# ZSHCRWY25/3DRVO-MARL-CollisionAvoidance

Hardware: AMD Instinct MI355X
Metric: drone-steps/sec (env.step throughput) (higher is better)
Workload: dtype f64; 1 GPU; BASELINE config 3 env.step: 64 drones x 4096 envs per GPU, nm=10, 0 buildings, map [50.0, 50.0, 10.0], fused step+auto-reset, f32 actions in HBM; envs_per_gpu=4096, drones=64, diag_build=False, cold_all=False, ablate=0, device_error_word=0

## Files before the change

3drvo-marl-collisionavoidance_amd/csrc/rvo3d_aux_kernels.hpp:

```cpp
#pragma once

#include "rvo3d_step.hpp"
#include "rvo3d_rvo_rules.hpp"

namespace rvo3d {

__device__ __forceinline__ void reset_drone(const Params& P, int g) {
  double s[3];
  load_wp(P, g, 0, s);
  P.px()[g] = s[0]; P.py()[g] = s[1]; P.pz()[g] = s[2];
  P.vx()[g] = 0.0; P.vy()[g] = 0.0; P.vz()[g] = 0.0;
  P.wp_idx()[g] = 1; P.arrive()[g] = 0; P.dest()[g] = 0;
  P.real_len()[g] = 0.0; P.max_dev()[g] = 0.0; P.yaw()[g] = 0.0; P.pitch()[g] = 0.0;
  double c1[3];
  load_wp(P, g, 1, c1);
  store3(P.cur(0), P.cur(1), P.cur(2), g, c1);
  store3(P.prev(0), P.prev(1), P.prev(2), g, s);
  const bool plain = P.dev0()[g] == 0.0;
  P.dvk_a()[g] = plain ? P.dv0_a()[g] : kDvInvalid;
  P.dvk_b()[g] = P.dv0_b()[g];
}
__global__ void reset_kernel(const Params P, const uint8_t* env_mask, const uint8_t* drone_mask) {
  const int g = blockIdx.x * blockDim.x + threadIdx.x;
  if (g >= P.E * P.N) return;
  if (env_mask && !env_mask[g / P.N]) return;
  if (drone_mask && !drone_mask[g]) return;
  reset_drone(P, g);
}

__global__ void reset_fresh_kernel(const Params P, const uint8_t* env_mask) {
  const int g = blockIdx.x * blockDim.x + threadIdx.x;
  if (g >= P.E * P.N) return;
  if (!env_mask[g / P.N]) return;
  reset_drone(P, g);
  P.extra_len()[g] = 0.0;
}

__global__ void wpcache_kernel(const Params P) {
  const int g = blockIdx.x * blockDim.x + threadIdx.x;
  if (g >= P.E * P.N) return;
  const int np = P.n_points()[g];
  int i = P.wp_idx()[g];
  i = i < 1 ? 1 : (i > np - 1 ? np - 1 : i);
  double v[3];
  load_wp(P, g, i, v);
  store3(P.cur(0), P.cur(1), P.cur(2), g, v);
  load_wp(P, g, i - 1, v);
  store3(P.prev(0), P.prev(1), P.prev(2), g, v);
}

__device__ __forceinline__ void dv0_drone(const Params& P, int g) {
  double p[3], cur[3], dv[3];
  load_wp(P, g, 0, p);
  load_wp(P, g, 1, cur);
  des_vel(P, p, cur, dv);
  uint32_t a, b;
  dv_encode(dv, a, b);
  P.dv0_a()[g] = a; P.dv0_b()[g] = b;
  P.dev0()[g] = deviation(p, cur, p);
}
__global__ void dv0_kernel(const Params P) {
  const int g = blockIdx.x * blockDim.x + threadIdx.x;
  if (g >= P.E * P.N) return;
  dv0_drone(P, g);
}

__device__ __forceinline__ int live_drones(const Params& P, int e) { return P.cold().counts[e]; }

template <bool CNT>
__device__ __forceinline__ void des_vel_body(const Params P, double* out) {
  const int g = blockIdx.x * blockDim.x + threadIdx.x;
  if (g >= P.E * P.N) return;
  if (CNT) {
    const int e = g / P.N;
    if (g - e * P.N >= live_drones(P, e)) {
      out[3 * (size_t)g] = 0.0; out[3 * (size_t)g + 1] = 0.0; out[3 * (size_t)g + 2] = 0.0;
      return;
    }
  }
  double p[3] = {P.px()[g], P.py()[g], P.pz()[g]}, cur[3], dv[3];
  load3(P.cur(0), P.cur(1), P.cur(2), g, cur);
  des_vel(P, p, cur, dv);
  out[3 * (size_t)g] = dv[0]; out[3 * (size_t)g + 1] = dv[1]; out[3 * (size_t)g + 2] = dv[2];
}
__global__ void des_vel_kernel(const Params P, double* out) { des_vel_body<false>(P, out); }
__global__ void des_vel_counted_kernel(const Params P, double* out) { des_vel_body<true>(P, out); }

struct RvoVelArgs { double vmax[3]; double acceler; };

__device__ __forceinline__ int arange_len(double lo, double hi) {
  const double n = __builtin_ceil((hi - lo) / 0.5);
  return n > 0 ? (int)n : 0;
}
__device__ __forceinline__ double arange_at(double lo, int k) {
  const double next = lo + 0.5;
  return k == 0 ? lo : (k == 1 ? next : lo + k * (next - lo));
}


__device__ __forceinline__ unsigned long long rvo_grid(const RvoVelArgs& A, const double* v0, double* lo, int* cnt) {
#pragma unroll
  for (int k = 0; k < 3; ++k) {
    lo[k] = clampd(v0[k] - A.acceler, -A.vmax[k], A.vmax[k]);
    const double hi = clampd(v0[k] + A.acceler, -A.vmax[k], A.vmax[k]);
    cnt[k] = arange_len(lo[k], hi);
    if (cnt[k] > 4) cnt[k] = 4;
  }
  unsigned long long live = 0ull;
  int c = 0;
  for (int ix = 0; ix < cnt[0]; ++ix)
    for (int iy = 0; iy < cnt[1]; ++iy)
      for (int iz = 0; iz < cnt[2]; ++iz, ++c)
// ... 134 lines not shown
```

3drvo-marl-collisionavoidance_amd/csrc/rvo3d_host_setup.hpp:

```cpp
#pragma once

#include "../../include/rvo3d.h"
#include "rvo3d_params.hpp"
#include "rvo3d_lds.hpp"

#include <cmath>
#include <cstring>
#include <string>
#include <vector>

namespace rvo3d {

inline size_t align_up(size_t x, size_t a) { return (x + a - 1) / a * a; }
inline volatile double kTwo = 2.0;
inline double py_sq(double x) { return std::pow(x, kTwo); }

inline double sq_threshold(double tau) {
  volatile double x = tau * tau;
  while (std::sqrt(std::nextafter((double)x, INFINITY)) <= tau) x = std::nextafter((double)x, INFINITY);
  while (std::sqrt((double)x) > tau) x = std::nextafter((double)x, -INFINITY);
  return x;
}

struct Pick { int nfix; bool pad; };
// ... 113 lines not shown
  two_phase = epb == P.epb && out.threads == G.threads;
  return RVO3D_OK;
}

inline int zero_fill_tables(const Params& P, int threads, Cold& C, std::string& err) {
  const int N = P.N, epb = P.epb;
  C.zf_div = (uint32_t)((P.W & 1) == 0 ? (P.W - 12) / 2 : (P.W - 12));
  C.zf_magic = 0;
  if (C.zf_div > 0) {
    const uint32_t m = (uint32_t)(((1ull << 32) + C.zf_div - 1) / C.zf_div);
    bool ok = true;
    const uint64_t qmax = (uint64_t)threads * C.zf_div;
    for (uint64_t q = 0; q < qmax && ok; ++q) ok = ((q * m) >> 32) == q / C.zf_div;
    if (!ok) {
      err = "neighbors_num too large for the zero-fill index trick";
      return RVO3D_ERR_INVALID;
    }
    C.zf_magic = m;
  }
  C.zf_q = (P.W & 1) == 0 ? (uint32_t)(P.W / 2) : 0u;
  C.zf_iters = 0;
  static_assert(kMaxThreads / 4 <= sizeof(C.zmask) / sizeof(C.zmask[0]),
                "Cold::zmask has one word per thread quad of the largest workgroup");
  std::memset(C.zmask, 0, sizeof C.zmask);
  {
    const uint32_t rb = 4u * (uint32_t)P.W;
    const uint32_t rows_full = (uint32_t)epb * (uint32_t)N, nwv = (uint32_t)threads / 64u;
    const uint32_t nblk = rows_full * rb >> 6;
    const uint32_t iters = (nblk + 16u * nwv - 1u) / (16u * nwv);
    if (C.zf_q != 0 && P.W >= 48 && (rows_full & 7u) == 0 && iters <= 32u) {
      for (uint32_t tq = 0; tq < (uint32_t)threads / 4u; ++tq) {
        uint32_t m = 0;
        for (uint32_t i = 0; i < iters; ++i) {
          const uint32_t blk = tq + 16u * nwv * i;
          if (blk >= nblk) break;
          const uint32_t o = (blk * 64u) % rb;
          if (o >= 48u && o + 64u <= rb) m |= 1u << i;
        }
        C.zmask[tq] = m;
      }
      C.zf_iters = (int)iters;
    }
  }
  return RVO3D_OK;
}

inline int plan_env(const rvo3d_config* cfg, int lds_pad, Params& P, Cold& C, Geometry& G, std::string& err) {
  std::memset(&P, 0, sizeof P);
  std::memset(&C, 0, sizeof C);
  P.E = cfg->num_envs; P.N = cfg->num_drones; P.P = cfg->max_points;
  C.nb = cfg->num_buildings; P.nm = cfg->neighbors_num; P.env_train = cfg->env_train ? 1 : 0;
  P.W = 12 + 9 * P.nm;
  C.act_scale = cfg->action_decimals >= 0 ? std::pow(10.0, cfg->action_decimals) : 0.0;
  for (int k = 0; k < 3; ++k) C.map[k] = cfg->map_size[k];
  P.T10 = sq_threshold(10.0);
  C.T5 = sq_threshold(5.0);
  building_grid_dims(cfg, C);
  C.T04 = sq_threshold(0.4);
  filter_bands(P, C);
  if (int rc = launch_geometry(lds_pad, P, G, err)) return rc;
  return zero_fill_tables(P, G.threads, C, err);
}

struct StagedWorld { std::vector<double> wp, rl, rad, pri, p95; };
inline int stage_world(Params& P, const double* waypoints, const int32_t* n_points, const double* radius,
                       const double* priority, StagedWorld& w, std::string& err) {
  const size_t EN = (size_t)P.E * P.N;
  std::vector<double> wp((size_t)P.P * 3 * EN), rl(EN), rad(EN), pri(EN), p95(P.P);
  for (size_t g = 0; g < EN; ++g) {
    const int np = n_points[g];
    if (np < 2 || np > P.P) {
      err = "n_points entries must be in [2, max_points]";
      return RVO3D_ERR_INVALID;
    }
    const double* src = waypoints + g * P.P * 3;
    double total = 0.0;
    for (int k = 0; k < P.P; ++k) {
      const int kk = k < np ? k : np - 1;
      for (int c = 0; c < 3; ++c) wp[((size_t)k * 3 + c) * EN + g] = src[kk * 3 + c];
      if (k + 1 < np) {
        const double dx = src[(k + 1) * 3] - src[k * 3], dy = src[(k + 1) * 3 + 1] - src[k * 3 + 1],
                     dz = src[(k + 1) * 3 + 2] - src[k * 3 + 2];
        total += std::sqrt(py_sq(dx) + py_sq(dy) + py_sq(dz));
      }
    }
    rl[g] = total;
    rad[g] = radius ? radius[g] : 0.2;
    pri[g] = priority ? priority[g] : 5.0;
  }
  {
    bool uni = true;
    for (size_t g = 1; g < EN && uni; ++g)
      uni = std::memcmp(&rad[g], &rad[0], 8) == 0 && std::memcmp(&pri[g], &pri[0], 8) == 0;
    P.uniform_rp = uni ? 1 : 0;
    P.r0 = rad[0];
    P.prio0 = pri[0];
  }
  for (int k = 0; k < P.P; ++k) p95[k] = std::pow(0.95, (double)k);
  w.wp.swap(wp); w.rl.swap(rl); w.rad.swap(rad); w.pri.swap(pri); w.p95.swap(p95);
  return RVO3D_OK;
}

inline double largest_radius(const std::vector<double>& rad) {
  double rmax = 0.0;
  for (size_t g = 0; g < rad.size(); ++g) {
    if (rad[g] != rad[g]) rmax = INFINITY;
// ... 161 lines not shown
```

3drvo-marl-collisionavoidance_amd/csrc/rvo3d_math.hpp:

```cpp
#pragma once

#include "rvo3d_params.hpp"

namespace rvo3d {

__device__ __forceinline__ double sq(double x) { return x * x; }
__device__ __forceinline__ double dot3b(double ax, double ay, double az, double bx,
                                        double by, double bz) {
  return __builtin_fma(az, bz, __builtin_fma(ay, by, ax * bx));
}
__device__ __forceinline__ double norm3b(double x, double y, double z) {
  return __builtin_sqrt(dot3b(x, y, z, x, y, z));
}
__device__ __forceinline__ double norm2sq(double x, double y) { return __builtin_fma(y, y, x * x); }
__device__ __forceinline__ bool finite_d(double q) { return __builtin_fabs(q) < __builtin_inf(); }

__device__ __forceinline__ float round2_f32(double x) {
  const double k = __builtin_rint(x * 100.0);
  return __builtin_fabs(k) < 16777216.0 ? (float)(k * 0.01) : (float)(k / 100.0);
}
__device__ __forceinline__ double k_over_1000(double k) {
  const double q = k * 0.001;
  const double r = __builtin_fma(-q, 1000.0, k);
  const double c = q + r * 0.001;
  return finite_d(k) ? c : k;
}

constexpr uint32_t kDvInvalid = 0xffffffffu;
__device__ __forceinline__ void dv_encode(const double dv[3], uint32_t& a, uint32_t& b) {
  const double k0 = __builtin_rint(dv[0] * 1000.0), k1 = __builtin_rint(dv[1] * 1000.0),
               k2 = __builtin_rint(dv[2] * 1000.0);
  const bool ok = __builtin_fabs(k0) <= 1023.0 && __builtin_fabs(k1) <= 1023.0 &&
                  __builtin_fabs(k2) <= 1023.0 && k_over_1000(k0) == dv[0] &&
                  k_over_1000(k1) == dv[1] && k_over_1000(k2) == dv[2];
  const uint32_t nz = (uint32_t)(k0 == 0.0 && __builtin_signbit(dv[0])) |
                      ((uint32_t)(k1 == 0.0 && __builtin_signbit(dv[1])) << 1) |
                      ((uint32_t)(k2 == 0.0 && __builtin_signbit(dv[2])) << 2);
  a = ok ? ((uint32_t)((int)k0 + 1024) | ((uint32_t)((int)k1 + 1024) << 16)) : kDvInvalid;
  b = (uint32_t)((int)(ok ? k2 : 0.0) + 1024) | (nz << 16);
}
__device__ __forceinline__ bool dv_decode(uint32_t a, uint32_t b, double dv[3]) {
  if (a == kDvInvalid) return false;
  const int k0 = (int)(a & 0xffffu) - 1024, k1 = (int)(a >> 16) - 1024, k2 = (int)(b & 0xffffu) - 1024;
  dv[0] = (b & (1u << 16)) ? -0.0 : k_over_1000((double)k0);
  dv[1] = (b & (1u << 17)) ? -0.0 : k_over_1000((double)k1);
  dv[2] = (b & (1u << 18)) ? -0.0 : k_over_1000((double)k2);
  return true;
}

__device__ __forceinline__ double py_round2_c(double x) {
  double p = x * 100.0;
  double e = __builtin_fma(x, 100.0, -p);
  double c = __builtin_floor(p);
  double d = (p - (c + 0.5)) + e;
  if (d > 0.0) c += 1.0;
  else if (d == 0.0 && (((long long)c) & 1)) c += 1.0;
  return c;
}
__device__ __forceinline__ double clampd(double x, double lo, double hi) {
  return x < lo ? lo : (x > hi ? hi : x);
}
__device__ __forceinline__ double np_mod(double a, double b) {
  double m;
  if (b > 0.0 && a > -b && a < 2.0 * b) m = a >= b ? a - b : a;
  else m = fmod(a, b);
  if (m != 0.0) {
    if ((b < 0.0) != (m < 0.0)) m += b;
  } else {
    m = __builtin_copysign(0.0, b);
  }
  return m;
}

__device__ __forceinline__ void des_vel(double T04, const double p[3], const double cur[3], double out[3]) {
  const double dx = cur[0] - p[0], dy = cur[1] - p[1], dz = cur[2] - p[2];
  const double d2 = dot3b(dx, dy, dz, dx, dy, dz);
  if (d2 > T04) {
    const double inv = 1000.0 / __builtin_sqrt(d2);
    const double ux = dx * inv, uy = dy * inv, uz = dz * inv;
    double kx = __builtin_rint(ux), ky = __builtin_rint(uy), kz = __builtin_rint(uz);
    const double m = __builtin_fmin(__builtin_fmin(0.5 - __builtin_fabs(ux - kx),
                                                   0.5 - __builtin_fabs(uy - ky)),
                                    0.5 - __builtin_fabs(uz - kz));
    if (!(m > 1e-7)) {
      const double az = atan2(dy, dx);
      const double el = atan2(dz, __builtin_sqrt(norm2sq(dx, dy)));
      double sa, ca, se, ce;
      sincos(az, &sa, &ca);
      sincos(el, &se, &ce);
      kx = __builtin_rint((1.0 * (ca * ce)) * 1000.0);
      ky = __builtin_rint((1.0 * (sa * ce)) * 1000.0);
      kz = __builtin_rint((1.0 * se) * 1000.0);
    }
    out[0] = k_over_1000(kx); out[1] = k_over_1000(ky); out[2] = k_over_1000(kz);
  } else {
    out[0] = out[1] = out[2] = 0.0;
  }
}
__device__ __forceinline__ void des_vel(const Params& P, const double p[3], const double cur[3],
                                        double out[3]) {
  des_vel(P.cold().T04, p, cur, out);
}

__device__ __forceinline__ double deviation(const double a[3], const double b[3],
                                            const double p[3]) {
  double dx = b[0] - a[0], dy = b[1] - a[1], dz = b[2] - a[2];
  double mag = __builtin_sqrt(sq(dx) + sq(dy) + sq(dz));
  if (mag == 0.0) return 0.0;
  double hx = dx / mag, hy = dy / mag, hz = dz / mag;
  double qx0 = p[0] - a[0], qy0 = p[1] - a[1], qz0 = p[2] - a[2];
  double t = qx0 * hx + qy0 * hy + qz0 * hz;
  double qx = a[0] + t * hx, qy = a[1] + t * hy, qz = a[2] + t * hz;
  return __builtin_sqrt(sq(p[0] - qx) + sq(p[1] - qy) + sq(p[2] - qz));
}

__device__ __forceinline__ bool arrived(double T04, const double p[3], const double d[3]) {
  const double x = p[0] - d[0], y = p[1] - d[1], z = p[2] - d[2];
  return dot3b(x, y, z, x, y, z) <= T04;
}

__device__ __forceinline__ double vo_exp_time(double rx, double ry, double rz, double rvx,
                                              double rvy, double rvz, double ra, double rb) {
  double r = ra + rb;
  double ux = -rvx, uy = -rvy, uz = -rvz;
  double a = sq(ux) + sq(uy) + sq(uz);
  double b = 2 * rx * ux + 2 * ry * uy + 2 * rz * uz;
  double c = sq(rx) + sq(ry) + sq(rz) - sq(r);
  if (c <= 0) return 0.0;
  double temp = sq(b) - 4 * a * c;
  if (temp <= 0) return __builtin_inf();
  double s = __builtin_sqrt(temp);
  double t1 = (-b + s) / (2 * a);
  double t2 = (-b - s) / (2 * a);
  if (t1 < 0 && t2 < 0) return -1.0;
  double t3 = t1 >= 0 ? t1 : __builtin_inf();
  double t4 = t2 >= 0 ? t2 : __builtin_inf();
  return t4 < t3 ? t4 : t3;
}

struct Drone {
  double x, y, z, vx, vy, vz, r, prio;
};

struct PairOut {
  bool collision, flag;
  double t, iet, md;
  int alpha_c;
};

}
```

3drvo-marl-collisionavoidance_amd/csrc/rvo3d_params.hpp:

```cpp
#pragma once

#include <hip/hip_runtime.h>
#include <stdint.h>

namespace rvo3d {

constexpr double kExpRadius = 0.2;
constexpr double kCtimeThreshold = 2.0;
constexpr double kDeg2Rad = 0.017453292519943295;
constexpr double kPi = 3.141592653589793;
constexpr int kMaxThreads = 512;
constexpr double kCosD = 0.999999995;
constexpr double kSinD = 1.0000000000e-4;

struct Cold {
  double map[3];
  double T5, T04;
  double cen[3];
  double act_scale;
  float cmax;
  float kdot;
  uint32_t zf_div;
  uint32_t zf_magic;
  uint32_t zf_q;
  int zf_iters;
  uint32_t zmask[128];
  int nb;
  const double* bld;
  const double* pow95;
  const uint16_t* bgrid;
  int bgx, bgy;
  double bg_inv;
  uint32_t bld_stride, bgrid_stride;
  const int32_t* counts;
  int cnt_two_phase;
};
constexpr int kBgridK = 15;
typedef const __attribute__((address_space(4))) Cold ColdC;

struct Params {
  int E, N, P, nm, env_train, epb, W;
  int action_f64;
  int dv_cached;
  int g_cached;
  int action_mode;
  float acceler;
#ifdef RVO3D_DIAG
  int ablate;
#endif
  int zf16;
  int uniform_rp;
  double r0, prio0;
  double T10;
  float t10n;
  float bandn;
  float band;
  int nw;
  float x1_gap;
  float x1_k2;
  float x1_cs2;
  double* f64;
  int32_t* i32;
  uint8_t* u8;
  uint32_t S;
  enum { F_PX, F_PY, F_PZ, F_VX, F_VY, F_VZ, F_YAW, F_PITCH, F_REAL_LEN, F_MAX_DEV, F_EXTRA_LEN,
         F_CUR, F_PREV = F_CUR + 3,
         F_ROUTE_LEN = F_PREV + 3, F_RADIUS, F_PRIO, F_DEV0, F_WP };
  __host__ __device__ double* f(int k) const { return f64 + (size_t)k * S; }
  __host__ __device__ double* px() const { return f(F_PX); }
  __host__ __device__ double* py() const { return f(F_PY); }
  __host__ __device__ double* pz() const { return f(F_PZ); }
  __host__ __device__ double* vx() const { return f(F_VX); }
  __host__ __device__ double* vy() const { return f(F_VY); }
  __host__ __device__ double* vz() const { return f(F_VZ); }
  __host__ __device__ double* yaw() const { return f(F_YAW); }
  __host__ __device__ double* pitch() const { return f(F_PITCH); }
  __host__ __device__ double* real_len() const { return f(F_REAL_LEN); }
  __host__ __device__ double* max_dev() const { return f(F_MAX_DEV); }
  __host__ __device__ double* extra_len() const { return f(F_EXTRA_LEN); }
  __host__ __device__ int32_t* wp_idx() const { return i32; }
  __host__ __device__ uint8_t* arrive() const { return u8; }
  __host__ __device__ uint8_t* dest() const { return u8 + S; }
  __host__ __device__ double* route_len() const { return f(F_ROUTE_LEN); }
  __host__ __device__ double* radius() const { return f(F_RADIUS); }
  __host__ __device__ double* prio() const { return f(F_PRIO); }
  __host__ __device__ double* dev0() const { return f(F_DEV0); }
  __host__ __device__ double* wp(int k, int c) const { return f(F_WP + 3 * k + c); }
  __host__ __device__ double* cur(int c) const { return f(F_CUR + c); }
  __host__ __device__ double* prev(int c) const { return f(F_PREV + c); }
  __host__ __device__ int32_t* n_points() const { return i32 + S; }
  __host__ __device__ uint32_t* dvk_a() const { return reinterpret_cast<uint32_t*>(i32) + (size_t)2 * S; }
  __host__ __device__ uint32_t* dvk_b() const { return reinterpret_cast<uint32_t*>(i32) + (size_t)3 * S; }
  __host__ __device__ uint32_t* dv0_a() const { return reinterpret_cast<uint32_t*>(i32) + (size_t)4 * S; }
  __host__ __device__ uint32_t* dv0_b() const { return reinterpret_cast<uint32_t*>(i32) + (size_t)5 * S; }
  __host__ __device__ uint32_t* gcache(int w) const { return reinterpret_cast<uint32_t*>(i32) + (size_t)(6 + w) * S; }
  __host__ __device__ double* row_iet(int s) const { return f(F_WP + 3 * P + s); }
  __host__ __device__ uint32_t* row_pk(int s) const {
    return reinterpret_cast<uint32_t*>(i32) + (size_t)(6 + nw + s) * S;
  }
  __host__ __device__ static size_t f64_arrays(int P_, int nm_) { return F_WP + 3 * (size_t)P_ + (nm_ > 0 ? nm_ : 1); }
  __host__ __device__ static size_t i32_arrays(int nm_, int nw_) { return 6 + (size_t)nw_ + (size_t)(nm_ > 0 ? nm_ : 1); }
  uint32_t* err;
  const Cold* cold_;
  __device__ __forceinline__ ColdC& cold() const { return *(ColdC*)cold_; }
#ifdef RVO3D_DIAG
  unsigned long long* dbg;
#endif
  const void* actions;
  float* obs;
  int32_t* vo_count;
  float* reward;
  double* reward64;
  uint8_t *done, *info, *finish, *reset_mask;
  const int32_t* prev_cnt;
};

#ifdef RVO3D_DIAG
#define RVO3D_STAMP(i)                                                                  \
  do {                                                                                  \
    if (P.dbg && threadIdx.x == 0) P.dbg[(size_t)blockIdx.x * 32 + (i)] = __builtin_amdgcn_s_memtime(); \
  } while (0)
#define RVO3D_ABLATED(bits) ((P.ablate & (bits)) != 0)
#else
#define RVO3D_STAMP(i) do { } while (0)
#define RVO3D_ABLATED(bits) false
#endif

}
```

3drvo-marl-collisionavoidance_amd/csrc/rvo3d_step.hpp:

```cpp
#pragma once

#include "rvo3d_pairs.hpp"

namespace rvo3d {

__device__ __forceinline__ bool building_test(const double* const bld, int b, const Drone& S,
                                              double T5) {
  const double bx = bld[4 * b], by = bld[4 * b + 1], bh = bld[4 * b + 2], br = bld[4 * b + 3];
  const double ex = S.x - bx, ey = S.y - by;
  if ((bh > S.z - 2) & (norm2sq(ex, ey) <= T5) & (S.z <= bh))
    return __builtin_sqrt(sq(ex) + sq(ey)) <= S.r + br;
  return false;
}
__device__ __forceinline__ bool building_hit(const Params& P, const Drone& S, int e) {
  const int nb = P.cold().nb;
  if (nb == 0) return false;
  bool hit = false;
  const double* const bld = P.cold().bld + (size_t)e * P.cold().bld_stride;
  const double T5 = P.cold().T5;
  const int gx = P.cold().bgx;
  if (gx > 0) {
    const int gy = P.cold().bgy;
    const double inv = P.cold().bg_inv;
    int ix = (int)__builtin_floor(S.x * inv), iy = (int)__builtin_floor(S.y * inv);
// ... 167 lines not shown
#pragma unroll
    for (int u = 0; u < 4; ++u)
      if ((m >> u) & 1u) {
        *reinterpret_cast<v4f*>(p + u * step) = (v4f){0.f, 0.f, 0.f, 0.f};
      }
  }
}

template <int NW>
__device__ __forceinline__ void late_row_windows(const Params& P, const Lds& L, int tid, int row0,
                                                 int nrows) {
  const uint32_t rb = 4u * (uint32_t)P.W, q = rb >> 3;
  const int ln = tid & 63, wv = tid >> 6;
  const int nwv = waves_of<NW>(L);
  const float2* pro2 = reinterpret_cast<const float2*>(L.w[0]);
  char* const base = reinterpret_cast<char*>(P.obs) + (size_t)row0 * rb;
  const int ch = ln & 7;
  const int r0 = wv * 8 + (ln >> 3);
  const uint32_t rs0 = rb * (uint32_t)r0;
  const uint32_t s8 = (rs0 & 63u) >> 3;
  const uint32_t ua = 2u * (uint32_t)ch, ub = ua + 1u;
  const bool pa = ua < s8, pb = ub < s8;
  const uint32_t uia = pa ? q - s8 + ua : ua - s8, uib = pb ? q - s8 + ub : ub - s8;
  const bool proa = uia < 6u, prob = uib < 6u;
  const int pia = (int)(proa ? uia : 5u), pib = (int)(prob ? uib : 5u);
  const int da_row = pa ? 1 : 0, db_row = pb ? 1 : 0;
  char* pc = base + (rs0 & ~63u) + 16u * (uint32_t)ch;
  const size_t step = (size_t)8 * (size_t)nwv * rb;
  for (int r = r0; r < nrows; r += 8 * nwv, pc += step) {
    const int ra = r - da_row, rbw = r - db_row;
    const int za = L.kept[ra], zb = L.kept[rbw];
    const float2 da = pro2[ra * 6 + pia], db = pro2[rbw * 6 + pib];
    const bool va = proa | (uia >= (uint32_t)za), vb = prob | (uib >= (uint32_t)zb);
    const float2 a = proa ? da : make_float2(0.f, 0.f), b = prob ? db : make_float2(0.f, 0.f);
    if (va & vb) *reinterpret_cast<float4*>(pc) = make_float4(a.x, a.y, b.x, b.y);
    if (va != vb) *reinterpret_cast<float2*>(pc + (vb ? 8 : 0)) = vb ? b : a;
  }
}

__device__ __forceinline__ void write_vo_rows(const Params& P, const Lds& L, int tid, int lbase,
                                              int g, const Drone& S, int kept) {
  float* o = P.obs + (size_t)g * P.W;
  bool bad = false;
  for (int s = 0; s < kept; ++s) {
    const uint32_t pk = P.row_pk(s)[g];
    const int j = (int)(pk & 0xffffu);
    const Drone O = lds_drone(L, lbase + j);
    const double pr = (S.prio == O.prio) ? 0.5 : S.prio / (S.prio + O.prio);
    double row[9];
    row[0] = pr * (2 * S.x + (S.vx + O.vx));
    row[1] = pr * (2 * S.y + (S.vy + O.vy));
    row[2] = pr * (2 * S.z + (S.vz + O.vz));
    row[3] = O.x - S.x; row[4] = O.y - S.y; row[5] = O.z - S.z;
    row[6] = (double)(pk >> 16) / 100.0;
    row[7] = pair_md(S, O);
    row[8] = P.row_iet(s)[g];
#pragma unroll
    for (int k = 0; k < 9; ++k) {
      bad |= !finite_d(row[k]);
      o[12 + 9 * s + k] = round2_f32(row[k]);
    }
  }
  P.vo_count[g] = kept;
  if (bad) atomicOr(P.err, 1u);
}

__device__ __forceinline__ void publish_zero_run(const Params& P, int g, int kept) {
  if ((P.W & 1) == 0 && ((9 * kept) & 1) && kept < P.nm) P.obs[(size_t)g * P.W + 12 + 9 * kept] = 0.0f;
}

__device__ __forceinline__ int live_count(const Params& P, int e) {
  return ((const __attribute__((address_space(4))) int32_t*)P.cold().counts)[e];
}
__device__ __forceinline__ void ghost_row(const Params& P, const Lds& L, int lrow, int g) {
  P.vo_count[g] = 0;
  if (P.zf16) {
    float4* pro = reinterpret_cast<float4*>(L.w[0]) + 3 * lrow;
    pro[0] = pro[1] = pro[2] = make_float4(0.f, 0.f, 0.f, 0.f);
    L.kept[lrow] = 6;
  } else {
    float* o = P.obs + (size_t)g * P.W;
#pragma unroll
    for (int k = 0; k < 12; ++k) o[k] = 0.0f;
    L.kept[lrow] = 0;
  }
}
__device__ __forceinline__ void ghost_outputs(const Params& P, int g, bool lite) {
  P.reward[g] = 0.0f;
  if (P.reward64) P.reward64[g] = 0.0;
  P.done[g] = 0; P.info[g] = 0; P.finish[g] = 0;
  if (lite && P.reset_mask) P.reset_mask[g] = 0;
}

__device__ __forceinline__ void zero_fill(const Params& P, const Lds& L, int tid, int row0,
                                          int nrows) {
  const uint32_t per_row = P.cold().zf_div;
  if (per_row == 0) return;
  const uint32_t total = (uint32_t)nrows * per_row;
  float* base = P.obs + (size_t)row0 * P.W + 12;
  if ((P.W & 1) == 0) {
    for (uint32_t q = tid; q < total; q += L.T) {
      const uint32_t row = (uint32_t)(((uint64_t)q * P.cold().zf_magic) >> 32);
      const uint32_t c = q - row * per_row;
      const uint32_t first = (9u * (uint32_t)L.kept[row] + 1u) >> 1;
      if (c >= first)
        *reinterpret_cast<float2*>(base + (size_t)row * P.W + 2 * c) = make_float2(0.f, 0.f);
    }
// ... 106 lines not shown
```

3drvo-marl-collisionavoidance_amd/csrc/rvo3d_step_body.hpp:

```cpp
  extern __shared__ __attribute__((aligned(16))) unsigned char smem[];
  Params P = Pin;
  static_assert(!PAD || NFIX != 0, "a padded kernel has a compile-time ring size");
  const int Nr = Pin.N;
  if (NFIX) { P.N = NFIX; P.epb = NFIX <= 64 ? 64 / NFIX : 1; }
  const int tid = threadIdx.x, T = (NW == 1 || NFIX) ? 64 * NW : (int)blockDim.x, N = P.N;
  const Lds L = carve_lds(smem, T, P.nm, P.epb, N, NW);
  const int el = tid / N;
  const int d = tid - el * N;
  const int e0 = blockIdx.x * P.epb;
  const int e = e0 + el;
  static_assert(!CNT || PAD, "per-env counts run on the padded kernels");
  const int Nl = CNT ? (((el < P.epb) && (e < P.E)) ? live_count(P, e) : Nr) : Nr;
  const bool active = (el < P.epb) && (e < P.E) && (!PAD || d < Nl);
  const bool ghost_in = CNT ? ((el < P.epb) && (e < P.E) && d >= Nl && d < Nr) : false;
  const bool rowed = CNT ? (active || ghost_in) : active;
  const int g = rowed ? e * (PAD ? Nr : N) + d : 0;
  const int lbase = el * N;
  const int full_rows = P.epb * (PAD ? Nr : N);
  const int nrows = ((P.E - e0) < P.epb ? (P.E - e0) : P.epb) * (PAD ? Nr : N);
  const int row0 = e0 * (PAD ? Nr : N);
  const int lrow = PAD ? el * Nr + d : tid;
  constexpr bool LITE = (MODE == kStepAutoReset);
  constexpr bool GSH = NW > 1 && NFIX == 64 * NW;
  constexpr bool XQ = NW == 1 && NFIX != 0;

  RVO3D_STAMP(0);
  Drone S;
  S.x = S.y = S.z = S.vx = S.vy = S.vz = 0.0; S.r = 0.2; S.prio = 5;
  if (PAD && d >= Nl) {
    S.x = S.y = S.z = __builtin_inf();
    const int o = el * 2 * N + d, os = el * N + d;
#pragma unroll
    for (int k = 0; k < 12; ++k) {
      const float v = (k == WX || k == WY || k == WZ) ? 1e30f : (k == WKD ? -1.0f : 0.0f);
      if (k == WX || k == WY || k == WZ || k == WR) {
        L.w[k][o] = v;
        if (d <= (N >> 1)) L.w[k][o + N] = v;
      } else L.w[k][os] = v;
    }
  }
  double a[3] = {0, 0, 0}, cur[3] = {0, 0, 0}, dv[3] = {0, 0, 0};
  double dev = 0, max_dev = 0;
  int wpi = 1;

  uint32_t gw[NW];
  const bool have_gw = MODE != kObserve && P.g_cached != 0;
  uint32_t old_cnt = 0;
  const bool act_f64 = P.action_mode != 1 && P.action_f64 != 0;
  float af[3] = {0.f, 0.f, 0.f};
  double ad[3] = {0, 0, 0};
  if (active) {
    if (LITE && NW == 1 && P.prev_cnt) old_cnt = (uint32_t)P.prev_cnt[g];
    S.x = P.px()[g]; S.y = P.py()[g]; S.z = P.pz()[g];
    S.vx = P.vx()[g]; S.vy = P.vy()[g]; S.vz = P.vz()[g];
    if (P.uniform_rp) { S.r = P.r0; S.prio = P.prio0; }
    else { S.r = P.radius()[g]; S.prio = P.prio()[g]; }
    if (have_gw) {
#pragma unroll
      for (int w = 0; w < NW; ++w) gw[w] = P.gcache(w)[g];
    }
    if (MODE != kObserve) {
      if (act_f64) {
        const double* A = static_cast<const double*>(P.actions) + (size_t)g * 3;
        ad[0] = A[0]; ad[1] = A[1]; ad[2] = A[2];
      } else {
        const float* A = static_cast<const float*>(P.actions) + (size_t)g * 3;
        af[0] = A[0]; af[1] = A[1]; af[2] = A[2];
      }
      if (P.action_mode == 1) {
        const double vv[3] = {S.vx, S.vy, S.vz};
#pragma unroll
        for (int k = 0; k < 3; ++k) {
          const float r = __builtin_rintf(af[k] * 100.0f) / 100.0f;
          const double x = (double)(P.acceler * r) + vv[k];
          a[k] = __builtin_rint(x * 100.0) / 100.0;
        }
      } else {
#pragma unroll
        for (int k = 0; k < 3; ++k) a[k] = act_f64 ? ad[k] : (double)af[k];
        const double act_scale = P.cold().act_scale;
        if (act_scale > 0) {
          a[0] = __builtin_rint(a[0] * act_scale) / act_scale;
          a[1] = __builtin_rint(a[1] * act_scale) / act_scale;
          a[2] = __builtin_rint(a[2] * act_scale) / act_scale;
        }
      }
    }
  }
  if (CNT && ghost_in && LITE && NW == 1 && P.prev_cnt) old_cnt = (uint32_t)P.prev_cnt[g];
  RVO3D_STAMP(1);
  double az[3] = {a[0], a[1], a[2]};
  if (norm3b(a[0], a[1], a[2]) < 1e-5) az[0] = az[1] = az[2] = 0.0;
  const double zero3[3] = {0, 0, 0};

  if (tid < P.epb) { L.any_reset[tid] = 0; L.far[tid] = 0; }
  if (LITE && NW > 1 && tid == 0) *L.any_old = 0;
  L.kept[tid] = 0;
  __syncthreads();
  if (LITE && NW == 1 && rowed && P.prev_cnt) L.kept[lrow] = clamp_kept(P, old_cnt);
  L.x[tid] = S.x; L.y[tid] = S.y; L.z[tid] = S.z;
  L.vx[tid] = S.vx; L.vy[tid] = S.vy; L.vz[tid] = S.vz;
  L.r[tid] = S.r; L.prio[tid] = S.prio;
  {
    const double p[3] = {S.x, S.y, S.z}, v[3] = {S.vx, S.vy, S.vz};
    stage_f32<NW>(P, L, el, d, active, p, v, az, S.r, S.prio);
  }
  __syncthreads();

  bool flag, collision = false;
  double tmin;

  if (MODE == kObserve) {
    if (active) {
      double prev[3];
      max_dev = P.max_dev()[g];
      load3(P.cur(0), P.cur(1), P.cur(2), g, cur);
      load3(P.prev(0), P.prev(1), P.prev(2), g, prev);
      const double p[3] = {S.x, S.y, S.z};
      des_vel(P, p, cur, dv);
      dev = deviation(prev, cur, p);
      if (dev > max_dev) max_dev = dev;
    }
    const int kept = sweep_env<NW, true, true, TRAIN, GSH, XQ>(P, L, tid, el, d, g, active, S, zero3, true, true, flag,
                                               tmin, collision, gw, false);
    if (active) {
      write_vo_rows(P, L, tid, lbase, g, S, kept);
      if (P.zf16) stage_row(P, L, lrow, g, S, proprio_tail(dv, dev), kept);
      else {
        write_proprio(P, g, S, proprio_tail(dv, dev));
        publish_zero_run(P, g, kept);
        L.kept[lrow] = kept;
      }
      P.max_dev()[g] = max_dev;
      uint32_t dvk_a, dvk_b;
      dv_encode(dv, dvk_a, dvk_b);
      P.dvk_a()[g] = dvk_a; P.dvk_b()[g] = dvk_b;
#pragma unroll
      for (int w = 0; w < NW; ++w) P.gcache(w)[g] = gw[w];
    }
    if (CNT && ghost_in) ghost_row(P, L, lrow, g);
    __syncthreads();
    if (P.zf16) row_fill_pairs<NW>(P, L, tid, row0, nrows);
    else zero_fill(P, L, tid, row0, nrows);
    return;
  }

  RVO3D_STAMP(2);
  sweep_env<NW, false, false, TRAIN, GSH, XQ>(P, L, tid, el, d, g, active && !RVO3D_ABLATED(1), S, az, false, false, flag,
                              tmin, collision, gw, have_gw);
  double rew_k = 0;
  double mov_nc = 0;
  bool f_dest = false;
  RVO3D_STAMP(3);
  constexpr bool kLoadAhead = NW <= 2;
  double prev[3] = {0, 0, 0}, yaw = 0, pitch = 0, real_len = 0, route_len = 0;
  int npts = 2;
  bool f_arrive_in = false, f_dest_in = false;
  if (active) {
    max_dev = P.max_dev()[g];
    load3(P.cur(0), P.cur(1), P.cur(2), g, cur);
    uint32_t dvk_a = 0, dvk_b = 0;
    if (P.dv_cached) { dvk_a = P.dvk_a()[g]; dvk_b = P.dvk_b()[g]; }
    if (kLoadAhead) {
      wpi = P.wp_idx()[g]; load3(P.prev(0), P.prev(1), P.prev(2), g, prev);
      yaw = P.yaw()[g]; pitch = P.pitch()[g]; real_len = P.real_len()[g]; route_len = P.route_len()[g];
      npts = P.n_points()[g]; f_arrive_in = P.arrive()[g] != 0; f_dest_in = P.dest()[g] != 0;
    }
    bool have = false;
    if (P.dv_cached) have = dv_decode(dvk_a, dvk_b, dv);
    if (!have) {
      if (!kLoadAhead) load3(P.prev(0), P.prev(1), P.prev(2), g, prev);
      const double p[3] = {S.x, S.y, S.z};
      des_vel(P, p, cur, dv);
      dev = deviation(prev, cur, p);
      if (dev > max_dev) max_dev = dev;
    }
    rew_k = rvo_reward_k(rvo_reward_pre(dv, a), flag, tmin);
  }
  RVO3D_STAMP(18);
  __syncthreads();
  if (active) {
    if (!kLoadAhead) {
      wpi = P.wp_idx()[g]; load3(P.prev(0), P.prev(1), P.prev(2), g, prev);
      yaw = P.yaw()[g]; pitch = P.pitch()[g]; real_len = P.real_len()[g]; route_len = P.route_len()[g];
      npts = P.n_points()[g]; f_arrive_in = P.arrive()[g] != 0; f_dest_in = P.dest()[g] != 0;
    }
    bool ex_set = false;
    double extra_len = 0.0;
    const int wpi_in = wpi;
    bool f_arrive = f_arrive_in;
    f_dest = f_dest_in;

    double speed = norm3b(S.vx, S.vy, S.vz);
    const double acc = clampd(a[0] * 1.0, -1.0, 1.0);
    const double dyaw = clampd(a[1] * 90.0, -90.0, 90.0);
    const double dpit = clampd(a[2] * 90.0, -90.0, 90.0);
    const double nv = speed + acc;
    speed = (0.0 > nv) ? 0.0 : nv;
    yaw = np_mod(yaw + dyaw, 360.0);
    pitch = clampd(pitch + dpit, -90.0, 90.0);
    double nvx = 0.0, nvy = 0.0, nvz = 0.0;
    if (!f_dest) {
      double sy, cy, sp, cp;
      sincos(yaw * kDeg2Rad, &sy, &cy);
      sincos(pitch * kDeg2Rad, &sp, &cp);
      nvx = speed * cp * cy; nvy = speed * cp * sy; nvz = speed * sp;
    }
    const double q0 = S.x, q1 = S.y, q2 = S.z;
    S.x = S.x + nvx; S.y = S.y + nvy; S.z = S.z + nvz;
    S.vx = nvx; S.vy = nvy; S.vz = nvz;
    real_len = real_len + norm3b(S.x - q0, S.y - q1, S.z - q2);
    const double p[3] = {S.x, S.y, S.z};
    const double T04 = P.cold().T04;
    double dst[3] = {0, 0, 0};
    if (f_arrive || arrived(T04, p, cur)) load_wp(P, g, npts - 1, dst);
    if (arrived(T04, p, cur)) {
      const bool at_dst = arrived(T04, p, dst);
      if (at_dst) { extra_len = real_len - route_len; ex_set = true; }
      if (!at_dst && wpi < npts - 1) {
        wpi += 1;
        prev[0] = cur[0]; prev[1] = cur[1]; prev[2] = cur[2];
        load_wp(P, g, wpi, cur);
        store3(P.cur(0), P.cur(1), P.cur(2), g, cur);
        store3(P.prev(0), P.prev(1), P.prev(2), g, prev);
        f_arrive = false;
      }
    }
    des_vel(T04, p, cur, dv);
    dev = deviation(prev, cur, p);
    if (dev > max_dev) max_dev = dev;
    bool arrive_r = false, dest_r = false;
    const int waypoint_num = wpi;
    if (!f_arrive && arrived(T04, p, cur)) { f_arrive = true; arrive_r = true; }
    if (f_arrive) {
      if (arrived(T04, p, dst)) {
        extra_len = real_len - route_len;
        ex_set = true;
        if (!f_dest) { f_dest = true; dest_r = true; }
      }
    }
    const double exlen = real_len - route_len + 4;
    mov_nc = mov_reward_k(P, false, arrive_r, waypoint_num, npts - 1, dest_r, dev, exlen > 0,
                          exlen);
    RVO3D_STAMP(19);
    const double map_x = P.cold().map[0], map_y = P.cold().map[1], map_z = P.cold().map[2];
    collision = building_hit(P, S, e);
    if ((S.x < 0) | (S.x > map_x) | (S.y < 0) | (S.y > map_y) | (S.z < 0) | (S.z > map_z))
      collision = true;
    P.yaw()[g] = yaw; P.pitch()[g] = pitch; P.real_len()[g] = real_len;
    if (ex_set) P.extra_len()[g] = extra_len;
    if (wpi != wpi_in) P.wp_idx()[g] = wpi;
    if (f_arrive != f_arrive_in) P.arrive()[g] = f_arrive ? 1 : 0;
    if (f_dest != f_dest_in) P.dest()[g] = f_dest ? 1 : 0;
    P.info[g] = f_arrive ? 1 : 0;
    P.finish[g] = f_dest ? 1 : 0;
  }
  L.x[tid] = S.x; L.y[tid] = S.y; L.z[tid] = S.z;
  L.vx[tid] = S.vx; L.vy[tid] = S.vy; L.vz[tid] = S.vz;
  {
    const double p[3] = {S.x, S.y, S.z}, v[3] = {S.vx, S.vy, S.vz};
    stage_f32<NW>(P, L, el, d, active, p, v, az, S.r, S.prio);
  }
  __syncthreads();

  RVO3D_STAMP(4);
  int kept = 0;
  if (LITE) {
    if (collide_env<NW, TRAIN, GSH>(P, L, tid, el, d, active && !RVO3D_ABLATED(2), S, gw)) collision = true;
  } else {
    kept = sweep_env<NW, true, true, TRAIN, GSH, XQ>(P, L, tid, el, d, g, active && !RVO3D_ABLATED(2), S, az, false,
                                     false, flag, tmin, collision, gw, false);
  }
  bool do_reset = false;
  if (active) {
    const double rew64 = k_over_1000(rew_k) + k_over_1000(collision ? -50000.0 : mov_nc);
    P.reward[g] = (float)rew64;
    if (P.reward64) P.reward64[g] = rew64;
    P.done[g] = collision ? 1 : 0;
    do_reset = LITE && (collision || f_dest);
  }
  if (CNT && ghost_in) ghost_outputs(P, g, LITE);

  RVO3D_STAMP(5);
  if (LITE) {
    if (active && P.reset_mask) P.reset_mask[g] = do_reset ? 1 : 0;
    if (do_reset) L.any_reset[el] = 1;
    __syncthreads();
    double p[3] = {0, 0, 0}, rcur[3] = {0, 0, 0}, rdev = 0.0;
    uint32_t rdv_a = 0, rdv_b = 0;
    if (NW > 1 && rowed && P.prev_cnt) old_cnt = (uint32_t)P.prev_cnt[g];
    if (do_reset) {
      load_wp(P, g, 0, p);
      rdev = P.dev0()[g];
      load_wp(P, g, 1, rcur);
      rdv_a = P.dv0_a()[g]; rdv_b = P.dv0_b()[g];
    }
    if (NW > 1 && rowed && P.prev_cnt) {
      L.kept[lrow] = clamp_kept(P, old_cnt);
      if (old_cnt != 0) *L.any_old = 1;
    }
    RVO3D_STAMP(26);
    if (NW == 1 && RVO3D_TWO_PHASE_ROWS && !RVO3D_ABLATED(16)) early_zero_blocks<NW>(P, L, tid, row0, nrows);
    RVO3D_STAMP(27);
    if (do_reset) {
      const double T04r = P.cold().T04;
      S.x = p[0]; S.y = p[1]; S.z = p[2]; S.vx = S.vy = S.vz = 0.0;
      dev = rdev;
      cur[0] = rcur[0]; cur[1] = rcur[1]; cur[2] = rcur[2];
      if (!dv_decode(rdv_a, rdv_b, dv)) {
        des_vel(T04r, p, cur, dv);
        dev = deviation(p, cur, p);
      }
      store3(P.cur(0), P.cur(1), P.cur(2), g, cur);
      store3(P.prev(0), P.prev(1), P.prev(2), g, p);
      max_dev = dev > 0.0 ? dev : 0.0;
      P.wp_idx()[g] = 1; P.arrive()[g] = 0; P.dest()[g] = 0;
      P.real_len()[g] = 0.0; P.yaw()[g] = 0.0; P.pitch()[g] = 0.0;
      L.x[tid] = S.x; L.y[tid] = S.y; L.z[tid] = S.z;
      L.vx[tid] = 0.0; L.vy[tid] = 0.0; L.vz[tid] = 0.0;
      const double v0[3] = {0, 0, 0};
      stage_f32<NW>(P, L, el, d, true, p, v0, az, S.r, S.prio);
    }
    if (active && L.any_reset[el] != 0) {
      const int os = el * N + d;
      L.w[WAX][os] = 0.f; L.w[WAY][os] = 0.f; L.w[WAZ][os] = 0.f;
    }
  }
  if (active) {
    uint32_t dvk_a, dvk_b;
    dv_encode(dv, dvk_a, dvk_b);
    P.dvk_a()[g] = dvk_a; P.dvk_b()[g] = dvk_b;
  }
  const ProprioTail ptail = proprio_tail(dv, dev);
  if (active) P.max_dev()[g] = max_dev;
  if (LITE) {
    __syncthreads();
    RVO3D_STAMP(6);
    const bool env_reset = (active || (PAD && el < P.epb)) && (L.any_reset[el] != 0);
    bool c2 = false;
    const double aa[3] = {env_reset ? 0.0 : az[0], env_reset ? 0.0 : az[1], env_reset ? 0.0 : az[2]};
    bool have_gw2 = !env_reset;
    if (NW == 1) {
      const unsigned long long rlanes = __ballot(do_reset);
      if (L.far[el] != 0) {
        uint32_t valid[1];
        valid_offsets<1>(N, d, valid);
        gw[0] = valid[0];
      } else {
        gw[0] = regate_resets(P, L, tid, el, d, active, rlanes, gw[0]);
      }
      have_gw2 = true;
    }
    if (RVO3D_ABLATED(2)) have_gw2 = false;
    if (NW > 1 && RVO3D_TWO_PHASE_ROWS && !RVO3D_ABLATED(16)) early_zero_blocks<NW>(P, L, tid, row0, nrows);
    kept = sweep_env<NW, true, false, TRAIN, GSH, XQ>(P, L, tid, el, d, g, active && !RVO3D_ABLATED(4), S, aa,
                                      false, env_reset, flag, tmin, c2, gw, have_gw2);
  }
  RVO3D_STAMP(7);
  const bool two_phase = LITE && RVO3D_TWO_PHASE_ROWS;
  if (NW > 1 && two_phase) {
    asm volatile("s_waitcnt vmcnt(0)" ::: "memory");
    __syncthreads();
  }
  if (active) {
    if (!RVO3D_ABLATED(8)) {
      if (two_phase) asm volatile("s_waitcnt vmcnt(0)" ::: "memory");
      write_vo_rows(P, L, tid, lbase, g, S, kept);
// ... 23 lines not shown
```

Measured before the change: 8.087 billion drone-steps/s.

## Cache per-leg unit direction and replace divisions by reciprocal-multiply with correction

Adds per-drone stored unit leg direction (leg and leg0 fields), computed when waypoints advance or reset, so deviation() avoids a sqrt and three divides every step. Also replaces double divisions by 100 or act_scale with multiply-by-reciprocal plus an FMA correction, falling back to true division when values are out of range. This adds six f64 state arrays, so each step does more loads and, on waypoint changes, more stores. It also risks bit-exactness if the correction formula differs from IEEE division in edge cases.

```diff
diff --git a/3drvo-marl-collisionavoidance_amd/csrc/rvo3d_aux_kernels.hpp b/3drvo-marl-collisionavoidance_amd/csrc/rvo3d_aux_kernels.hpp
--- a/3drvo-marl-collisionavoidance_amd/csrc/rvo3d_aux_kernels.hpp
+++ b/3drvo-marl-collisionavoidance_amd/csrc/rvo3d_aux_kernels.hpp
@@ -16,6 +16,9 @@
   load_wp(P, g, 1, c1);
   store3(P.cur(0), P.cur(1), P.cur(2), g, c1);
   store3(P.prev(0), P.prev(1), P.prev(2), g, s);
+  double h[3];
+  load3(P.leg0(0), P.leg0(1), P.leg0(2), g, h);
+  store3(P.leg(0), P.leg(1), P.leg(2), g, h);
   const bool plain = P.dev0()[g] == 0.0;
   P.dvk_a()[g] = plain ? P.dv0_a()[g] : kDvInvalid;
   P.dvk_b()[g] = P.dv0_b()[g];
@@ -43,10 +46,13 @@
   int i = P.wp_idx()[g];
   i = i < 1 ? 1 : (i > np - 1 ? np - 1 : i);
   double v[3];
-  load_wp(P, g, i, v);
-  store3(P.cur(0), P.cur(1), P.cur(2), g, v);
+  double c[3];
+  load_wp(P, g, i, c);
+  store3(P.cur(0), P.cur(1), P.cur(2), g, c);
   load_wp(P, g, i - 1, v);
   store3(P.prev(0), P.prev(1), P.prev(2), g, v);
+  const LegDir L = leg_dir(v, c);
+  store3(P.leg(0), P.leg(1), P.leg(2), g, L.h);
 }
 
 __device__ __forceinline__ void dv0_drone(const Params& P, int g) {
@@ -58,6 +64,8 @@
   dv_encode(dv, a, b);
   P.dv0_a()[g] = a; P.dv0_b()[g] = b;
   P.dev0()[g] = deviation(p, cur, p);
+  const LegDir L = leg_dir(p, cur);
+  store3(P.leg0(0), P.leg0(1), P.leg0(2), g, L.h);
 }
 __global__ void dv0_kernel(const Params P) {
   const int g = blockIdx.x * blockDim.x + threadIdx.x;
diff --git a/3drvo-marl-collisionavoidance_amd/csrc/rvo3d_host_setup.hpp b/3drvo-marl-collisionavoidance_amd/csrc/rvo3d_host_setup.hpp
--- a/3drvo-marl-collisionavoidance_amd/csrc/rvo3d_host_setup.hpp
+++ b/3drvo-marl-collisionavoidance_amd/csrc/rvo3d_host_setup.hpp
@@ -189,6 +189,8 @@
   C.nb = cfg->num_buildings; P.nm = cfg->neighbors_num; P.env_train = cfg->env_train ? 1 : 0;
   P.W = 12 + 9 * P.nm;
   C.act_scale = cfg->action_decimals >= 0 ? std::pow(10.0, cfg->action_decimals) : 0.0;
+  C.act_scale_exact = (C.act_scale == 10.0 || C.act_scale == 100.0 || C.act_scale == 1000.0) ? 1 : 0;
+  C.inv_act_scale = C.act_scale_exact ? 1.0 / C.act_scale : 0.0;
   for (int k = 0; k < 3; ++k) C.map[k] = cfg->map_size[k];
   P.T10 = sq_threshold(10.0);
   C.T5 = sq_threshold(5.0);
diff --git a/3drvo-marl-collisionavoidance_amd/csrc/rvo3d_math.hpp b/3drvo-marl-collisionavoidance_amd/csrc/rvo3d_math.hpp
--- a/3drvo-marl-collisionavoidance_amd/csrc/rvo3d_math.hpp
+++ b/3drvo-marl-collisionavoidance_amd/csrc/rvo3d_math.hpp
@@ -24,6 +24,21 @@
   const double r = __builtin_fma(-q, 1000.0, k);
   const double c = q + r * 0.001;
   return finite_d(k) ? c : k;
+}
+constexpr double kOverScaleMax = 16777216.0;
+__device__ __forceinline__ double over_scale(double k, double scale, double inv) {
+  const double q = k * inv;
+  const double r = __builtin_fma(-q, scale, k);
+  return __builtin_copysign(q + r * inv, k);
+}
+__device__ __forceinline__ void over_scale3(double k[3], double scale, double inv, bool exact) {
+  const bool in_range = __builtin_fabs(k[0]) < kOverScaleMax && __builtin_fabs(k[1]) < kOverScaleMax &&
+                        __builtin_fabs(k[2]) < kOverScaleMax;
+  if (exact && __ballot(!in_range) == 0ull) {
+    k[0] = over_scale(k[0], scale, inv); k[1] = over_scale(k[1], scale, inv); k[2] = over_scale(k[2], scale, inv);
+  } else {
+    k[0] = k[0] / scale; k[1] = k[1] / scale; k[2] = k[2] / scale;
+  }
 }
 
 constexpr uint32_t kDvInvalid = 0xffffffffu;
@@ -113,6 +128,29 @@
   double qx = a[0] + t * hx, qy = a[1] + t * hy, qz = a[2] + t * hz;
   return __builtin_sqrt(sq(p[0] - qx) + sq(p[1] - qy) + sq(p[2] - qz));
 }
+struct LegDir {
+  double h[3];
+  __device__ __forceinline__ bool on_file() const { return h[0] == h[0]; }
+};
+__device__ __forceinline__ LegDir leg_dir(const double a[3], const double b[3]) {
+  double dx = b[0] - a[0], dy = b[1] - a[1], dz = b[2] - a[2];
+  double mag = __builtin_sqrt(sq(dx) + sq(dy) + sq(dz));
+  LegDir L;
+  if (mag == 0.0) { L.h[0] = __builtin_nan(""); L.h[1] = L.h[2] = 0.0; }
+  else { L.h[0] = dx / mag; L.h[1] = dy / mag; L.h[2] = dz / mag; }
+  return L;
+}
+__device__ __forceinline__ double deviation(const double a[3], const LegDir& L, const double p[3]) {
+  double hx = L.h[0], hy = L.h[1], hz = L.h[2];
+  double qx0 = p[0] - a[0], qy0 = p[1] - a[1], qz0 = p[2] - a[2];
+  double t = qx0 * hx + qy0 * hy + qz0 * hz;
+  double qx = a[0] + t * hx, qy = a[1] + t * hy, qz = a[2] + t * hz;
+  return __builtin_sqrt(sq(p[0] - qx) + sq(p[1] - qy) + sq(p[2] - qz));
+}
+__device__ __forceinline__ double deviation(const double a[3], const double b[3], const LegDir& L, const double p[3]) {
+  if (L.on_file()) return deviation(a, L, p);
+  return deviation(a, b, p);
+}
 
 __device__ __forceinline__ bool arrived(double T04, const double p[3], const double d[3]) {
   const double x = p[0] - d[0], y = p[1] - d[1], z = p[2] - d[2];
diff --git a/3drvo-marl-collisionavoidance_amd/csrc/rvo3d_params.hpp b/3drvo-marl-collisionavoidance_amd/csrc/rvo3d_params.hpp
--- a/3drvo-marl-collisionavoidance_amd/csrc/rvo3d_params.hpp
+++ b/3drvo-marl-collisionavoidance_amd/csrc/rvo3d_params.hpp
@@ -18,6 +18,8 @@
   double T5, T04;
   double cen[3];
   double act_scale;
+  double inv_act_scale;
+  int act_scale_exact;
   float cmax;
   float kdot;
   uint32_t zf_div;
@@ -65,7 +67,8 @@
   uint32_t S;
   enum { F_PX, F_PY, F_PZ, F_VX, F_VY, F_VZ, F_YAW, F_PITCH, F_REAL_LEN, F_MAX_DEV, F_EXTRA_LEN,
          F_CUR, F_PREV = F_CUR + 3,
-         F_ROUTE_LEN = F_PREV + 3, F_RADIUS, F_PRIO, F_DEV0, F_WP };
+         F_ROUTE_LEN = F_PREV + 3, F_RADIUS, F_PRIO, F_DEV0,
+         F_LEG, F_LEG0 = F_LEG + 3, F_WP = F_LEG0 + 3 };
   __host__ __device__ double* f(int k) const { return f64 + (size_t)k * S; }
   __host__ __device__ double* px() const { return f(F_PX); }
   __host__ __device__ double* py() const { return f(F_PY); }
@@ -88,6 +91,8 @@
   __host__ __device__ double* wp(int k, int c) const { return f(F_WP + 3 * k + c); }
   __host__ __device__ double* cur(int c) const { return f(F_CUR + c); }
   __host__ __device__ double* prev(int c) const { return f(F_PREV + c); }
+  __host__ __device__ double* leg(int c) const { return f(F_LEG + c); }
+  __host__ __device__ double* leg0(int c) const { return f(F_LEG0 + c); }
   __host__ __device__ int32_t* n_points() const { return i32 + S; }
   __host__ __device__ uint32_t* dvk_a() const { return reinterpret_cast<uint32_t*>(i32) + (size_t)2 * S; }
   __host__ __device__ uint32_t* dvk_b() const { return reinterpret_cast<uint32_t*>(i32) + (size_t)3 * S; }
diff --git a/3drvo-marl-collisionavoidance_amd/csrc/rvo3d_step.hpp b/3drvo-marl-collisionavoidance_amd/csrc/rvo3d_step.hpp
--- a/3drvo-marl-collisionavoidance_amd/csrc/rvo3d_step.hpp
+++ b/3drvo-marl-collisionavoidance_amd/csrc/rvo3d_step.hpp
@@ -243,7 +243,7 @@
     row[1] = pr * (2 * S.y + (S.vy + O.vy));
     row[2] = pr * (2 * S.z + (S.vz + O.vz));
     row[3] = O.x - S.x; row[4] = O.y - S.y; row[5] = O.z - S.z;
-    row[6] = (double)(pk >> 16) / 100.0;
+    row[6] = over_scale((double)(pk >> 16), 100.0, 0.01);
     row[7] = pair_md(S, O);
     row[8] = P.row_iet(s)[g];
 #pragma unroll
diff --git a/3drvo-marl-collisionavoidance_amd/csrc/rvo3d_step_body.hpp b/3drvo-marl-collisionavoidance_amd/csrc/rvo3d_step_body.hpp
--- a/3drvo-marl-collisionavoidance_amd/csrc/rvo3d_step_body.hpp
+++ b/3drvo-marl-collisionavoidance_amd/csrc/rvo3d_step_body.hpp
@@ -73,16 +73,17 @@
         for (int k = 0; k < 3; ++k) {
           const float r = __builtin_rintf(af[k] * 100.0f) / 100.0f;
           const double x = (double)(P.acceler * r) + vv[k];
-          a[k] = __builtin_rint(x * 100.0) / 100.0;
+          a[k] = __builtin_rint(x * 100.0);
         }
+        over_scale3(a, 100.0, 0.01, true);
       } else {
 #pragma unroll
         for (int k = 0; k < 3; ++k) a[k] = act_f64 ? ad[k] : (double)af[k];
         const double act_scale = P.cold().act_scale;
         if (act_scale > 0) {
-          a[0] = __builtin_rint(a[0] * act_scale) / act_scale;
-          a[1] = __builtin_rint(a[1] * act_scale) / act_scale;
-          a[2] = __builtin_rint(a[2] * act_scale) / act_scale;
+          a[0] = __builtin_rint(a[0] * act_scale); a[1] = __builtin_rint(a[1] * act_scale);
+          a[2] = __builtin_rint(a[2] * act_scale);
+          over_scale3(a, act_scale, P.cold().inv_act_scale, P.cold().act_scale_exact != 0);
         }
       }
     }
@@ -153,6 +154,9 @@
   bool f_dest = false;
   RVO3D_STAMP(3);
   constexpr bool kLoadAhead = NW <= 2;
+  constexpr bool kLegOnFile = kLoadAhead;
+  LegDir leg;
+  leg.h[0] = __builtin_nan(""); leg.h[1] = leg.h[2] = 0.0;
   double prev[3] = {0, 0, 0}, yaw = 0, pitch = 0, real_len = 0, route_len = 0;
   int npts = 2;
   bool f_arrive_in = false, f_dest_in = false;
@@ -163,6 +167,7 @@
     if (P.dv_cached) { dvk_a = P.dvk_a()[g]; dvk_b = P.dvk_b()[g]; }
     if (kLoadAhead) {
       wpi = P.wp_idx()[g]; load3(P.prev(0), P.prev(1), P.prev(2), g, prev);
+      if (kLegOnFile) load3(P.leg(0), P.leg(1), P.leg(2), g, leg.h);
       yaw = P.yaw()[g]; pitch = P.pitch()[g]; real_len = P.real_len()[g]; route_len = P.route_len()[g];
       npts = P.n_points()[g]; f_arrive_in = P.arrive()[g] != 0; f_dest_in = P.dest()[g] != 0;
     }
@@ -172,7 +177,7 @@
       if (!kLoadAhead) load3(P.prev(0), P.prev(1), P.prev(2), g, prev);
       const double p[3] = {S.x, S.y, S.z};
       des_vel(P, p, cur, dv);
-      dev = deviation(prev, cur, p);
+      dev = kLegOnFile ? deviation(prev, cur, leg, p) : deviation(prev, cur, p);
       if (dev > max_dev) max_dev = dev;
     }
     rew_k = rvo_reward_k(rvo_reward_pre(dv, a), flag, tmin);
@@ -223,11 +228,13 @@
         load_wp(P, g, wpi, cur);
         store3(P.cur(0), P.cur(1), P.cur(2), g, cur);
         store3(P.prev(0), P.prev(1), P.prev(2), g, prev);
+        if (kLegOnFile) { leg = leg_dir(prev, cur); store3(P.leg(0), P.leg(1), P.leg(2), g, leg.h); }
+        else P.leg(0)[g] = __builtin_nan("");
         f_arrive = false;
       }
     }
     des_vel(T04, p, cur, dv);
-    dev = deviation(prev, cur, p);
+    dev = kLegOnFile ? deviation(prev, cur, leg, p) : deviation(prev, cur, p);
     if (dev > max_dev) max_dev = dev;
     bool arrive_r = false, dest_r = false;
     const int waypoint_num = wpi;
@@ -288,12 +295,14 @@
     __syncthreads();
     double p[3] = {0, 0, 0}, rcur[3] = {0, 0, 0}, rdev = 0.0;
     uint32_t rdv_a = 0, rdv_b = 0;
+    double rleg[3] = {__builtin_nan(""), 0, 0};
     if (NW > 1 && rowed && P.prev_cnt) old_cnt = (uint32_t)P.prev_cnt[g];
     if (do_reset) {
       load_wp(P, g, 0, p);
       rdev = P.dev0()[g];
       load_wp(P, g, 1, rcur);
       rdv_a = P.dv0_a()[g]; rdv_b = P.dv0_b()[g];
+      if (kLegOnFile) load3(P.leg0(0), P.leg0(1), P.leg0(2), g, rleg);
     }
     if (NW > 1 && rowed && P.prev_cnt) {
       L.kept[lrow] = clamp_kept(P, old_cnt);
@@ -313,6 +322,8 @@
       }
       store3(P.cur(0), P.cur(1), P.cur(2), g, cur);
       store3(P.prev(0), P.prev(1), P.prev(2), g, p);
+      if (kLegOnFile) store3(P.leg(0), P.leg(1), P.leg(2), g, rleg);
+      else P.leg(0)[g] = __builtin_nan("");
       max_dev = dev > 0.0 ? dev : 0.0;
       P.wp_idx()[g] = 1; P.arrive()[g] = 0; P.dest()[g] = 0;
       P.real_len()[g] = 0.0; P.yaw()[g] = 0.0; P.pitch()[g] = 0.0;
```

Result: no change. 8.121 billion drone-steps/s (median of 5 runs) (+0.4%).
